# medivhna/TF_Face_Toolbox

Measured on AMD Instinct MI355X. Metric: images/sec (whole node), SphereFaceNet-20 112x112 bs512, higher is better.
Workload: dtype f32; 1 GPU; SphereFaceNet-20 + A-softmax training step, 112x112x3, global batch 512, 10575 classes, Momentum, fp32; global_batch=512, per_gpu_batch=512, parallelism=dp1

## Files before the change

### tf_face_toolbox_amd/csrc/api.hip

```cpp
#include <hip/hip_runtime.h>
#include <stdio.h>
#include <stdlib.h>
#include <string.h>

#include <initializer_list>

#include "../../include/fte.h"
#include "igemm.h"
#include "wgrad16.h"
#include "pw16.h"
#include "kernels.h"
#include "layers.h"
#include "wino.h"
#include "search.h"

namespace {

struct Pads { int out, before; };
inline Pads same_pads(int in, int k, int stride) {
    const int out = (in + stride - 1) / stride;
    int total = (out - 1) * stride + k - in;
    if (total < 0) total = 0;
    return {out, total / 2};
}
// ... 254 lines not shown
inline bool wino_wanted(int n, int h, int wd, int cin, int cout, int ksize, int stride, int op) {
    return !plan_bf16() && !g_plan_bn && wino_sized(n, h, wd, cin, cout, ksize, stride, op);
}
inline bool aligned16(std::initializer_list<const void*> ptrs) {
    uintptr_t v = 0;
    for (const void* q : ptrs) v |= (uintptr_t)q;
    return (v & 15) == 0;
}
struct WinoWs { size_t v_off, u_off, slab_off, total; };
inline WinoWs wino_ws(int n, int h, int wd, int cin, int cout, int op, size_t head) {
    const WinoGeom g = wino_geom(n, h, wd);
    WinoWs w;
    w.v_off = align_up(head);
    if (op == 0) {
        w.u_off = w.v_off + align_up(wino_pack_floats(g.M, cin) * 4);
        w.slab_off = w.total = w.u_off + align_up((size_t)16 * cin * cout * 4);
    } else if (op == 1) {
        w.u_off = w.v_off + align_up(wino_pack_floats(g.M, cout) * 4);
        w.slab_off = w.total = w.u_off + align_up((size_t)16 * cin * cout * 4);
    } else {
        w.u_off = w.v_off + align_up(wino_pack_floats(g.M, cin) * 4);
        w.slab_off = w.u_off;
        w.total = w.slab_off + align_up((size_t)wino_wgrad_splits(cin, cout) * 16 * cin * cout * 4);
    }
    return w;
}
}

extern "C" {

#ifndef FTE_SRC_SHA
#define FTE_SRC_SHA "unstamped"
#endif
const char* fte_version(void) { return "fte 0.2 gfx950 fp32-mfma src:" FTE_SRC_SHA; }
// ... 69 lines not shown
    p.A = (const float*)x;
    p.B = (const float*)w;
    p.c_ld = cout;
    p.Y = y; p.Z = z; p.R = res; p.bias = bias; p.alpha = alpha; p.Y16 = y16;
    p.R16 = res16; p.Z16 = z16;
    int bl = BL_KN;
    if (src16) {
        p.src16 = 1; p.b_ld = cin; bl = BL_NK;
        for (int t = 0; t < ksize * ksize; ++t) p.b_tapoff[t] = t * cout * cin;
    } else {
        p.b_ld = cout;
    }
    if (!set_bytes(&p, (size_t)n * h * wd * cin, (size_t)ksize * ksize * cin * cout, src16 ? 2 : 4)) return FTE_EINVAL;
    if (!src16 && !stat_part && y && wino_wanted(n, h, wd, cin, cout, ksize, stride, 0)) {
        WinoWs wl = wino_ws(n, h, wd, cin, cout, 0, 0);
        if (vpack) { wl.u_off = 0; wl.total = align_up((size_t)16 * cin * cout * 4); }
        if (ws && ws_bytes >= wl.total) {
            if (!aligned16({x, w, bias, alpha, res, z, y, ws, vpack})) return FTE_EINVAL;
            float* V = vpack ? vpack : (float*)((char*)ws + wl.v_off);
            float* U = (float*)((char*)ws + wl.u_off);
            hipError_t e = wino_transform_filter((const float*)w, U, cin, cout, 0, (hipStream_t)stream);
            if (e != hipSuccess) return (int)e;
            e = wino_transform_tiles((const float*)x, V, n, h, wd, cin, 0, (hipStream_t)stream, wino_fwd_small_tiles());
            if (e != hipSuccess) return (int)e;
            WinoMMParams q;
            memset(&q, 0, sizeof(q));
            q.V = V; q.U = U; q.K = cin; q.N = cout; q.g = wino_geom(n, h, wd);
            q.Y = y; q.Z = z; q.R = res; q.bias = bias; q.alpha = alpha;
            return rc(wino_mm(q, EPI_FWD, (hipStream_t)stream));
        }
    }
    if (vpack) return FTE_EWORKSPACE;
    RowPlan rp = plan_rows(p.M, p.N, p.K, ws != nullptr, false, EPI_FWD);
    if (rp.tail_mode >= 2 && ws_bytes < rp.pw_bytes) rp = plan_rows(p.M, p.N, p.K, false);
    if (stat_part) {
        if (rp.tail_mode == 2) return FTE_EINVAL;
        p.SP = stat_part;
        *stat_rows = (int)(rp.main_mtiles + rp.tail_mtiles);
    }
    return rc(launch_rows(p, rp, AL_MK, bl, EPI_FWD, 0, (float*)ws, (hipStream_t)stream));
}
int fte_conv2d_fwd(const float* x, const float* w, const float* bias, const float* alpha, const float* res,
                   float* z, float* y, int n, int h, int wd, int cin, int cout, int ksize, int stride,
// ... 155 lines not shown
        const WinoWs wl = wino_ws(n, h, wd, cin, cout, 1, 2 * half_w + SCRATCH_BYTES);
        if (ws && ws_bytes >= wl.total) {
            if (!aligned16({dz, w, addin, zprev, alpha_prev, raw, dzprev, ws})) return FTE_EINVAL;
            const bool part = zprev && (dalpha_prev || dbias_prev);
            float* V = (float*)((char*)ws + wl.v_off);
            float* U = (float*)((char*)ws + wl.u_off);
            hipError_t e = wino_transform_filter((const float*)w, U, cin, cout, 1, (hipStream_t)stream);
            if (e != hipSuccess) return (int)e;
            e = wino_transform_tiles((const float*)dz, V, n, h, wd, cout, 0, (hipStream_t)stream);
            if (e != hipSuccess) return (int)e;
            WinoMMParams q;
            memset(&q, 0, sizeof(q));
            q.V = V; q.U = U; q.K = cout; q.N = cin; q.g = g;
            q.ADD = addin; q.RAW = raw; q.Zin = zprev; q.alpha = alpha_prev; q.amod = cin; q.DZ = dzprev;
            q.PA = part ? (float*)ws : nullptr; q.PB = part ? (float*)((char*)ws + half_w) : nullptr;
            e = wino_mm(q, EPI_DGRAD, (hipStream_t)stream);
            if (e != hipSuccess) return (int)e;
            if (part) {
                float* scratch = (float*)((char*)ws + 2 * half_w);
                if (dalpha_prev && dbias_prev) return rc(k_reduce_rows2(q.PA, dalpha_prev, q.PB, dbias_prev, nullptr, 1, g.MB, cin, 1, 1.f, scratch, (hipStream_t)stream));
                if (dalpha_prev) return rc(k_reduce_rows(q.PA, dalpha_prev, nullptr, 1, g.MB, cin, 1, 1.f, scratch, (hipStream_t)stream));
                return rc(k_reduce_rows(q.PB, dbias_prev, nullptr, 1, g.MB, cin, 1, 1.f, scratch, (hipStream_t)stream));
            }
            return FTE_OK;
        }
    }
    DgradClass cls[4];
    const int nc = dgrad_classes(n, h, wd, cin, cout, ksize, stride, cls);
    const bool merged = dgrad_mergeable(cls, nc, n, cin);
    long rows = 0;
// ... 1144 lines not shown
```

### tf_face_toolbox_amd/csrc/wino.h

```cpp
#pragma once
#include <hip/hip_runtime.h>
#include <stddef.h>

struct WinoGeom {
    int n, h, w, th, tw;
    long M;
    int MB;
};
WinoGeom wino_geom(int n, int h, int w);

inline size_t wino_pack_floats(long rows, int c) { return (size_t)((rows + 63) / 64) * 64 * (size_t)c * 16; }

hipError_t wino_transform_tiles(const float* x, float* pack, int n, int h, int w, int c, int mode, hipStream_t st, bool small = false);
hipError_t wino_transform_filter(const float* w, float* pack, int cin, int cout, int dgrad, hipStream_t st);

struct WinoMMParams {
    const float* V;
    const float* U;
    int K, N;
    WinoGeom g;
    float* Y; float* Z; const float* R; const float* bias; const float* alpha;
    const float* ADD; float* RAW; const float* Zin; float* DZ; float* PA; float* PB;
    int amod;
};
hipError_t wino_mm(const WinoMMParams& p, int epi, hipStream_t st);

int wino_wgrad_splits(int cin, int cout);
hipError_t wino_wgrad(const float* V, const float* dz, float* slabs, float* dw, const WinoGeom& g, int cin, int cout, hipStream_t st);

void wino_set_algo(int a);
int wino_get_algo();
```

### tf_face_toolbox_amd/csrc/wino.hip

```cpp
#include <hip/hip_runtime.h>
#include <stdint.h>
#include <stdio.h>
#include <stdlib.h>
#include <string.h>

#include <atomic>

#include "igemm.h"
#include "igemm_dev.h"
#include "wino.h"

#ifdef FTE_WINO_STAMP
__device__ unsigned long long* g_wino_stamp = nullptr;
extern "C" int fte_debug_set_wino_stamp(void* buf) {
    return (int)hipMemcpyToSymbol(HIP_SYMBOL(g_wino_stamp), &buf, sizeof(buf));
}
#endif

namespace {

using namespace igemm_dev;

typedef __attribute__((address_space(3))) void lds_void;
__device__ __forceinline__ void dma16(const __amdgpu_buffer_rsrc_t& r, char* lds, unsigned voff, unsigned soff) {
// ... 85 lines not shown
        p[1][b] = 0.5f * (g[0][b] + g[1][b] + g[2][b]);
        p[2][b] = 0.5f * (g[0][b] - g[1][b] + g[2][b]);
        p[3][b] = g[2][b];
    }
    const int KS = K >> 3, rb = row >> 6, r = row & 63, c8 = k & 7;
    float* o = pack + ((((size_t)rb * KS + (k >> 3)) * 16) * 64 + r) * 8 + (((c8 >> 2) ^ ((r >> 4) & 1)) << 2) + (c8 & 3);
#pragma unroll
    for (int i = 0; i < 4; ++i) {
        o[(size_t)(4 * i + 0) * 512] = p[i][0];
        o[(size_t)(4 * i + 1) * 512] = 0.5f * (p[i][0] + p[i][1] + p[i][2]);
        o[(size_t)(4 * i + 2) * 512] = 0.5f * (p[i][0] - p[i][1] + p[i][2]);
        o[(size_t)(4 * i + 3) * 512] = p[i][2];
    }
}

template <int EPI, int NWN>
__global__ __launch_bounds__(256 * NWN, 1) void wino_mm_kernel(const WinoMMParams p, int NBX, int GRP, int vid0, int nvirt) {
    constexpr int NW = 4 * NWN;
    constexpr int BSTG = NWN * (SLAB_B / 2);
    constexpr int STG = SLAB_B + BSTG;
    extern __shared__ __attribute__((aligned(16))) char wsm[];
    const int tid = threadIdx.x;
    const int lane = tid & 63;
    const int wid = __builtin_amdgcn_readfirstlane(tid >> 6);
    const int q = wid & 1, mi = (wid >> 1) & 1, ni = NWN == 2 ? wid >> 2 : 0;
    const int hb = NWN == 2 ? 0 : (int)(blockIdx.x & 1);
    const int li = lane & 31, lh = lane >> 5;
    const int KS = p.K >> 3, NB = p.N >> 6;
    auto decode = [&](int vid, int& mb, int& nb) -> bool {
        if (GRP > 0) {
            const int xcd = vid & 7, slot = vid >> 3;
            const int grp = xcd % GRP, cls = xcd / GRP, C = 8 / GRP;
            mb = (slot / NBX) * C + cls;
            nb = grp * NBX + slot % NBX;
        } else {
            mb = vid / NB; nb = vid - mb * NB;
        }
        return mb < p.g.MB;
    };
    auto next_valid = [&](int vid, int& mb, int& nb) -> int {
        if constexpr (NWN == 2) {
            for (; vid < nvirt; vid += (int)gridDim.x)
                if (decode(vid, mb, nb)) return vid;
        } else if (vid == vid0) {
            int c = 0;
            for (int v = vid0; v < nvirt; ++v)
                if (decode(v, mb, nb)) {
                    if (c == (int)(blockIdx.x >> 1)) return v;
                    ++c;
                }
        }
        return nvirt;
    };
    const unsigned voff = (unsigned)lane * 16u;
    auto issue = [&](int mb, int nb, int s, int stage) {
        const __amdgpu_buffer_rsrc_t rsA = __builtin_amdgcn_make_buffer_rsrc(const_cast<float*>(p.V + (size_t)mb * KS * SLAB_F), 0, (unsigned)KS * SLAB_B, 0x00020000);
// ... 7 lines not shown
#pragma unroll
        for (int i = 0; i < 4; ++i) {
            const int piece = wid + NW * i;
            dma16(rsB, base + SLAB_B + piece * 1024, voff, (unsigned)(s * SLAB_B + (NWN == 2 ? piece : 2 * piece + hb) * 1024));
        }
    };
    constexpr int BPL = NWN * 1024;
    const int a_off = ((8 * q) * 64 + 32 * mi + li) * 32 + ((lh ^ ((li >> 4) & 1)) << 4);
    const int b_off = (8 * q) * BPL + (32 * ni + li) * 32 + ((lh ^ ((li >> 4) & 1)) << 4);
    float* xb = reinterpret_cast<float*>(wsm + STG);
    int* rowpix = reinterpret_cast<int*>(wsm + 2 * STG);
    int* rowflag = rowpix + 64;
    float* red = reinterpret_cast<float*>(rowflag + 64);

    int mb = 0, nb = 0;
    int vid = next_valid(NWN == 2 ? vid0 + (int)blockIdx.x : vid0, mb, nb);
    if (vid >= nvirt) return;
    f32x4 xa[4], xb4[4], ya[4], yb[4];
    auto read_frags = [&](int stage, int half, f32x4 (&fa)[4], f32x4 (&fb)[4], int t) {
        const char* As = wsm + stage * STG;
        fa[t] = *reinterpret_cast<const f32x4*>(As + a_off + (4 * half + t) * 2048);
        fb[t] = *reinterpret_cast<const f32x4*>(As + SLAB_B + b_off + (4 * half + t) * BPL);
    };
    auto dma_piece = [&](const __amdgpu_buffer_rsrc_t& rsA, const __amdgpu_buffer_rsrc_t& rsB, int s, int stage, int i) {
        char* base = wsm + stage * STG;
        if constexpr (NWN == 2) {
            const int piece = wid + 8 * (i >> 1);
            if (i & 1) dma16(rsB, base + SLAB_B + piece * 1024, voff, (unsigned)(s * SLAB_B + piece * 1024));
            else dma16(rsA, base + piece * 1024, voff, (unsigned)(s * SLAB_B + piece * 1024));
        } else {
            const int piece = wid + 4 * (i & 7);
            if (i >= 8) dma16(rsB, base + SLAB_B + piece * 1024, voff, (unsigned)(s * SLAB_B + (2 * piece + hb) * 1024));
            else dma16(rsA, base + piece * 1024, voff, (unsigned)(s * SLAB_B + piece * 1024));
        }
    };
    constexpr int NDMA = NWN == 2 ? 8 : 12;
    issue(mb, nb, 0, 0);
    issue(mb, nb, 1, 1);
    asm volatile("s_waitcnt vmcnt(0)\n\ts_barrier" ::: "memory");
#pragma unroll
    for (int t = 0; t < 4; ++t) read_frags(0, 0, xa, xb4, t);
    bool first = true;
    while (vid < nvirt) {
        int mb2 = 0, nb2 = 0;
        const int vid2 = NWN == 2 ? next_valid(vid + (int)gridDim.x, mb2, nb2) : nvirt;
        const bool has_next = vid2 < nvirt;
#ifdef FTE_WINO_STAMP
        unsigned long long st0 = 0, sr0 = 0, st1 = 0;
        if (g_wino_stamp) { st0 = __builtin_amdgcn_s_memtime(); sr0 = __builtin_amdgcn_s_memrealtime(); __builtin_amdgcn_s_waitcnt(0xC07F); }
#endif
        f32x16 acc[8];
#pragma unroll
        for (int t = 0; t < 8; ++t)
#pragma unroll
            for (int r = 0; r < 16; ++r) acc[t][r] = 0.f;
        for (int s = 0; s < KS; ++s) {
            const int st = s & 1;
            __builtin_amdgcn_sched_barrier(0);
            static_for<0, 16>([&](auto ic) {
                constexpr int idx = decltype(ic)::value, j = idx >> 2, t = idx & 3;
                acc[t] = __builtin_amdgcn_mfma_f32_32x32x2f32(xa[t][j], xb4[t][j], acc[t], 0, 0, 0);
                if constexpr (idx < 4 && !(WMM_ABL & 2)) read_frags(st, 1, ya, yb, idx);
                __builtin_amdgcn_sched_barrier(0);
            });
            if constexpr (WMM_ABL & 4) asm volatile("s_waitcnt vmcnt(0) lgkmcnt(0)" ::: "memory");
            else if (s == 0 && !first) asm volatile("s_waitcnt vmcnt(16) lgkmcnt(0)\n\ts_barrier" ::: "memory");
            else asm volatile("s_waitcnt vmcnt(0) lgkmcnt(0)\n\ts_barrier" ::: "memory");
            const bool same = s + 2 < KS;
            const bool dma = same || (has_next && s + 2 == KS);
            const int dmb = same ? mb : mb2, dnb = same ? nb : nb2, ds = same ? s + 2 : 0;
            const __amdgpu_buffer_rsrc_t rsA = __builtin_amdgcn_make_buffer_rsrc(const_cast<float*>(p.V + (size_t)dmb * KS * SLAB_F), 0, dma ? (unsigned)KS * SLAB_B : 0u, 0x00020000);
            const __amdgpu_buffer_rsrc_t rsB = __builtin_amdgcn_make_buffer_rsrc(const_cast<float*>(p.U + (size_t)dnb * KS * SLAB_F), 0, dma ? (unsigned)KS * SLAB_B : 0u, 0x00020000);
            if (s == 0 && tid < 64) {
                const int m = mb * 64 + tid;
                int pix = -1, fl = 0;
                if (m < (int)p.g.M) {
                    const int tpi = p.g.th * p.g.tw;
                    const int n = m / tpi, rem = m - n * tpi;
                    const int ty = rem / p.g.tw, tx = rem - ty * p.g.tw;
                    pix = (n * p.g.h + 2 * ty) * p.g.w + 2 * tx;
                    fl = ((2 * ty + 1 < p.g.h) ? 1 : 0) | ((2 * tx + 1 < p.g.w) ? 2 : 0);
                }
                rowpix[tid] = pix; rowflag[tid] = fl;
            }
            __builtin_amdgcn_sched_barrier(0);
            static_for<0, 16>([&](auto ic) {
                constexpr int idx = decltype(ic)::value, j = idx >> 2, t = idx & 3;
                acc[4 + t] = __builtin_amdgcn_mfma_f32_32x32x2f32(ya[t][j], yb[t][j], acc[4 + t], 0, 0, 0);
                if constexpr (idx < 4 && !(WMM_ABL & 2)) read_frags(st ^ 1, 0, xa, xb4, idx);
                if constexpr (idx >= 4 && idx < 4 + NDMA && !(WMM_ABL & 1)) dma_piece(rsA, rsB, ds, st, idx - 4);
                __builtin_amdgcn_sched_barrier(0);
            });
        }
#ifdef FTE_WINO_STAMP
        if (g_wino_stamp) { st1 = __builtin_amdgcn_s_memtime(); __builtin_amdgcn_s_waitcnt(0xC07F); }
#endif
        asm volatile("s_waitcnt vmcnt(0) lgkmcnt(0)\n\ts_barrier" ::: "memory");
// ... 4 lines not shown
        float keep[16][2];
#pragma unroll
        for (int r = 0; r < 16; ++r) {
            const float p00 = acc[0][r] + acc[1][r] + acc[2][r], p01 = acc[1][r] - acc[2][r] - acc[3][r];
            const float p10 = acc[4][r] + acc[5][r] + acc[6][r], p11 = acc[5][r] - acc[6][r] - acc[7][r];
            float s0, s1;
            if (q == 0) { keep[r][0] = p00 + p10; keep[r][1] = p01 + p11; s0 = p10; s1 = p11; }
            else { keep[r][0] = -p00 - p10; keep[r][1] = -p01 - p11; s0 = p00; s1 = p01; }
            xb[(wid * 32 + 2 * r) * 64 + lane_e] = s0;
            xb[(wid * 32 + 2 * r + 1) * 64 + lane_e] = s1;
        }
        __builtin_amdgcn_sched_barrier(0);
        const int prw = lane_e >> 3, pc4 = lane_e & 7;
        const int ch0 = nb * 64 + 32 * (NWN == 2 ? ni : hb) + 4 * pc4;
        unsigned off[2][2][2];
#pragma unroll
        for (int h2 = 0; h2 < 2; ++h2)
#pragma unroll
            for (int j = 0; j < 2; ++j) {
                const int rr = 32 * mi + 16 * h2 + prw + 8 * j;
                const int pix = rowpix[rr], fl = rowflag[rr];
                const bool rowok = pix >= 0 && (q == 0 || (fl & 1));
                const unsigned o = (unsigned)((pix + q * p.g.w) * p.N + ch0) * 4u;
                off[0][h2][j] = rowok ? o : OOB;
                off[1][h2][j] = (rowok && (fl & 2)) ? o + (unsigned)p.N * 4u : OOB;
            }
        const unsigned tbytes = (unsigned)((size_t)p.g.n * p.g.h * p.g.w * p.N * 4);
        auto rsrc_of = [&](const float* q_) { return __builtin_amdgcn_make_buffer_rsrc(const_cast<float*>(q_), 0, q_ ? tbytes : 0u, 0x00020000); };
        auto ld4 = [&](const __amdgpu_buffer_rsrc_t& r_, unsigned o) { return __builtin_bit_cast(f32x4, __builtin_amdgcn_raw_buffer_load_b128(r_, o, 0, 0)); };
        auto st4 = [&](const __amdgpu_buffer_rsrc_t& r_, unsigned o, const f32x4& v) { __builtin_amdgcn_raw_buffer_store_b128(__builtin_bit_cast(u32x4, v), r_, o, 0, 0); };
        f32x4 in0[2][2][2], in1[2][2][2];
        f32x4 bias4 = {0.f, 0.f, 0.f, 0.f}, al4 = {1.f, 1.f, 1.f, 1.f};
        bool act = false;
        if constexpr (EPI == EPI_FWD) {
            const __amdgpu_buffer_rsrc_t rsR = rsrc_of(p.R);
#pragma unroll
            for (int b = 0; b < 2; ++b)
#pragma unroll
                for (int h2 = 0; h2 < 2; ++h2)
#pragma unroll
                    for (int j = 0; j < 2; ++j) in0[b][h2][j] = ld4(rsR, off[b][h2][j]);
            if (p.bias) bias4 = *reinterpret_cast<const f32x4*>(p.bias + ch0);
            act = p.alpha != nullptr;
            if (act) al4 = *reinterpret_cast<const f32x4*>(p.alpha + ch0);
        } else {
            const __amdgpu_buffer_rsrc_t rsA = rsrc_of(p.ADD), rsZ = rsrc_of(p.Zin);
#pragma unroll
            for (int b = 0; b < 2; ++b)
#pragma unroll
                for (int h2 = 0; h2 < 2; ++h2)
#pragma unroll
                    for (int j = 0; j < 2; ++j) { in0[b][h2][j] = ld4(rsA, off[b][h2][j]); in1[b][h2][j] = ld4(rsZ, off[b][h2][j]); }
            act = p.Zin != nullptr;
            if (act) al4 = *reinterpret_cast<const f32x4*>(p.alpha + ch0 % p.amod);
        }
        asm volatile("s_waitcnt lgkmcnt(0)\n\ts_barrier" ::: "memory");
#pragma unroll
        for (int r = 0; r < 16; ++r)
#pragma unroll
            for (int b = 0; b < 2; ++b) keep[r][b] += xb[((wid ^ 1) * 32 + 2 * r + b) * 64 + lane_e];
        asm volatile("s_waitcnt lgkmcnt(0)\n\ts_barrier" ::: "memory");
        if (has_next) issue(mb2, nb2, 1, 1);
        float* patch = reinterpret_cast<float*>(wsm + 2 * STG + 2560) + wid * (16 * 36);
        f32x4 sa4 = {0.f, 0.f, 0.f, 0.f}, sb4 = {0.f, 0.f, 0.f, 0.f};
        const __amdgpu_buffer_rsrc_t rsO0 = rsrc_of(EPI == EPI_FWD ? p.Z : p.RAW), rsO1 = rsrc_of(EPI == EPI_FWD ? p.Y : p.DZ);
#pragma unroll
        for (int b = 0; b < 2; ++b)
#pragma unroll
            for (int h2 = 0; h2 < 2; ++h2) {
                __builtin_amdgcn_wave_barrier();
#pragma unroll
                for (int r8 = 0; r8 < 8; ++r8) patch[((r8 & 3) + 8 * (r8 >> 2) + 4 * lh_e) * 36 + li_e] = keep[8 * h2 + r8][b];
                __builtin_amdgcn_fence(__ATOMIC_RELEASE, "wavefront");
                __builtin_amdgcn_wave_barrier();
#pragma unroll
                for (int j = 0; j < 2; ++j) {
                    f32x4 v = *reinterpret_cast<const f32x4*>(patch + (prw + 8 * j) * 36 + 4 * pc4);
                    const unsigned o = off[b][h2][j];
                    if constexpr (EPI == EPI_FWD) {
                        v += bias4;
                        st4(rsO0, o, v);
#pragma unroll
                        for (int e = 0; e < 4; ++e) v[e] = v[e] > 0.f ? v[e] : al4[e] * v[e];
                        v += in0[b][h2][j];
                        st4(rsO1, o, v);
                    } else {
                        v += in0[b][h2][j];
                        st4(rsO0, o, v);
                        const bool in = o != OOB;
#pragma unroll
                        for (int e = 0; e < 4; ++e) {
                            const float z = act ? in1[b][h2][j][e] : 1.f;
                            sa4[e] += in ? v[e] * fminf(z, 0.f) : 0.f;
                            v[e] *= prelu_slope(z, al4[e]);
                            sb4[e] += in ? v[e] : 0.f;
                        }
                        st4(rsO1, o, v);
                    }
                }
            }
        if constexpr (EPI == EPI_DGRAD) {
            if (p.PA) {
#pragma unroll
                for (int e = 0; e < 4; ++e) {
                    float a_ = sa4[e], b_ = sb4[e];
                    a_ += __shfl_xor(a_, 8); b_ += __shfl_xor(b_, 8);
                    a_ += __shfl_xor(a_, 16); b_ += __shfl_xor(b_, 16);
                    a_ += __shfl_xor(a_, 32); b_ += __shfl_xor(b_, 32);
                    if (prw == 0) { red[wid * 32 + 4 * pc4 + e] = a_; red[(NW + wid) * 32 + 4 * pc4 + e] = b_; }
                }
                asm volatile("s_waitcnt lgkmcnt(0)\n\ts_barrier" ::: "memory");
                if (tid < 32 * NWN) {
                    const int n2 = tid >> 5, l2 = tid & 31;
                    float a = 0.f, b = 0.f;
#pragma unroll
                    for (int k = 0; k < 4; ++k) { a += red[(4 * n2 + k) * 32 + l2]; b += red[(NW + 4 * n2 + k) * 32 + l2]; }
                    const size_t o = (size_t)mb * p.N + nb * 64 + (NWN == 2 ? tid : 32 * hb + tid);
                    p.PA[o] = a;
                    if (p.PB) p.PB[o] = b;
                }
            }
        }
#ifdef FTE_WINO_STAMP
        if (g_wino_stamp && tid == 0) {
            const unsigned long long t2 = __builtin_amdgcn_s_memtime(), r2 = __builtin_amdgcn_s_memrealtime();
            unsigned long long* o = g_wino_stamp + 8 * (size_t)vid;
            o[0] = st1 - st0; o[1] = t2 - st1; o[2] = t2 - st0; o[3] = r2 - sr0; o[4] = sr0; o[5] = (unsigned long long)KS; o[6] = blockIdx.x; o[7] = r2;
        }
#endif
        if (has_next) {
#pragma unroll
            for (int t = 0; t < 4; ++t) read_frags(0, 0, xa, xb4, t);
        }
        vid = vid2; mb = mb2; nb = nb2;
        first = false;
    }
}

#ifndef WG_ABL
#define WG_ABL 0
#endif
constexpr int WG_KSTRIDE = 4096 + 32;
constexpr int WG_OP = 8 * WG_KSTRIDE;
__global__ __launch_bounds__(512, 1) void wino_wgrad_kernel(const float* __restrict__ V, const float* __restrict__ dz, float* __restrict__ slabs,
                                                            int cin, int cout, WinoGeom g, int S, unsigned dz_bytes) {
    extern __shared__ __attribute__((aligned(16))) char wsm[];
    const int tid = threadIdx.x;
    const int lane = tid & 63;
    const int wid = __builtin_amdgcn_readfirstlane(tid >> 6);
    const int li = lane & 31, lh = lane >> 5;
// ... 171 lines not shown
    const dim3 grid(8 * ((g.MB + 7) / 8) * (small ? 2 : 1), c / 32);
    if (mode == 0 && small) hipLaunchKernelGGL((wino_tiles_kernel<0, 256>), grid, dim3(256), 0, st, x, pack, h, w, c, g.th, g.tw, g.M, g.MB, (unsigned)xb);
    else if (mode == 0) hipLaunchKernelGGL((wino_tiles_kernel<0, 512>), grid, dim3(512), 0, st, x, pack, h, w, c, g.th, g.tw, g.M, g.MB, (unsigned)xb);
    else hipLaunchKernelGGL((wino_tiles_kernel<1, 512>), grid, dim3(512), 0, st, x, pack, h, w, c, g.th, g.tw, g.M, g.MB, (unsigned)xb);
    return hipGetLastError();
}

hipError_t wino_transform_filter(const float* w, float* pack, int cin, int cout, int dgrad, hipStream_t st) {
    if (cin % 64 || cout % 64) return hipErrorInvalidValue;
    const int total = cin * cout;
    hipLaunchKernelGGL(wino_filter_kernel, dim3((total + 255) / 256), dim3(256), 0, st, w, pack, cin, cout, dgrad);
    return hipGetLastError();
}

namespace {
template <int EPI, int NWN>
hipError_t wino_mm_launch(const WinoMMParams& p, int NBX, int GRP, int vid0, int vid1, int grid, int tiles, hipStream_t st) {
    constexpr int NW = 4 * NWN;
    const size_t lds = 2 * ((size_t)SLAB_B + NWN * (SLAB_B / 2)) + 2560 + (size_t)NW * 16 * 36 * 4;
    static std::atomic<unsigned> attr{0u};
    int dev = 0;
    (void)hipGetDevice(&dev);
    const unsigned bit = 1u << (dev & 31);
    if (!(attr.load(std::memory_order_acquire) & bit)) {
        hipError_t e = hipFuncSetAttribute(reinterpret_cast<const void*>(wino_mm_kernel<EPI, NWN>), hipFuncAttributeMaxDynamicSharedMemorySize, (int)lds);
        if (e != hipSuccess) return e;
        attr.fetch_or(bit, std::memory_order_release);
    }
    const int sig[5] = {AL_MK, BL_NK, EPI, 8, 1};
    const double frac = (double)tiles / ((double)p.g.MB * (p.N / 64));
    const double flops = 2.0 * 16.0 * (double)tiles * 64.0 * 64.0 * p.K;
    const double bytes = frac * ((double)wino_pack_floats(p.g.M, p.K) * 4.0 + 16.0 * p.N * p.K * 4.0 + (double)p.g.n * p.g.h * p.g.w * p.N * 4.0 *
                                 (EPI == EPI_FWD ? (1 + (p.Z ? 1 : 0) + (p.R ? 1 : 0)) : (1 + (p.ADD ? 1 : 0) + (p.RAW ? 1 : 0) + (p.Zin ? 1 : 0))));
    const int h = igemm_prof_begin(sig, (int)((long)tiles * 64 / (p.N / 64)), p.N, 16 * p.K, flops, bytes, st);
    hipLaunchKernelGGL((wino_mm_kernel<EPI, NWN>), dim3(grid), dim3(256 * NWN), lds, st, p, NBX, GRP, vid0, vid1);
    igemm_prof_end(h, EPI == EPI_FWD ? (NWN == 2 ? "wino_mm_kernel<0,2>" : "wino_mm_kernel<0,1>") : (NWN == 2 ? "wino_mm_kernel<1,2>" : "wino_mm_kernel<1,1>"), st);
    return hipGetLastError();
}
}

hipError_t wino_mm(const WinoMMParams& p, int epi, hipStream_t st) {
    if (p.K % 64 || p.N % 64 || p.g.MB <= 0) return hipErrorInvalidValue;
    if ((size_t)p.g.n * p.g.h * p.g.w * p.N >= ((size_t)1 << 31)) return hipErrorInvalidValue;
    const int NB = p.N / 64;
    int NBX = NB < 2 ? NB : 2, GRP = NB / NBX;
    static const int plain = getenv("FTE_WINO_PLAIN_ORDER") ? atoi(getenv("FTE_WINO_PLAIN_ORDER")) : 0;
    int nvirt;
    if (plain || NB % NBX || 8 % GRP) { GRP = 0; nvirt = p.g.MB * NB; }
    else { const int C = 8 / GRP; nvirt = 8 * ((p.g.MB + C - 1) / C) * NBX; }
    static int cus = 0;
    if (!cus) {
        int dev = 0;
// ... 1 lines not shown
        if (hipGetDevice(&dev) != hipSuccess || hipGetDeviceProperties(&prop, dev) != hipSuccess) return hipErrorInvalidDevice;
        cus = prop.multiProcessorCount > 8 ? prop.multiProcessorCount / 8 * 8 : 8;
    }
    const int grid = nvirt < cus ? (nvirt + 7) / 8 * 8 : cus;
    static const int halves = getenv("FTE_WINO_HALF_TILES") ? atoi(getenv("FTE_WINO_HALF_TILES")) : 1;
    auto valid = [&](int vid) {
        if (GRP > 0) { const int xcd = vid & 7, slot = vid >> 3, cls = xcd / GRP, C = 8 / GRP; return (slot / NBX) * C + cls < p.g.MB; }
        return vid / NB < p.g.MB;
    };
    const int rounds = (nvirt + grid - 1) / grid, last = grid * (rounds - 1);
    int L = 0;
    for (int v = last; v < nvirt; ++v) L += valid(v) ? 1 : 0;
    const int total = p.g.MB * NB;
    int tail_base = nvirt;
    if (halves && L > 0 && 2 * L <= cus && (rounds == 1 || halves == 2)) tail_base = last;
    hipError_t e = hipSuccess;
    if (tail_base > 0) {
        e = epi == EPI_FWD ? wino_mm_launch<EPI_FWD, 2>(p, NBX, GRP, 0, tail_base, grid, total - (tail_base < nvirt ? L : 0), st)
                           : wino_mm_launch<EPI_DGRAD, 2>(p, NBX, GRP, 0, tail_base, grid, total - (tail_base < nvirt ? L : 0), st);
        if (e != hipSuccess) return e;
    }
    if (tail_base < nvirt)
        e = epi == EPI_FWD ? wino_mm_launch<EPI_FWD, 1>(p, NBX, GRP, tail_base, nvirt, 2 * L, L, st)
                           : wino_mm_launch<EPI_DGRAD, 1>(p, NBX, GRP, tail_base, nvirt, 2 * L, L, st);
    return e;
}

int wino_wgrad_splits(int cin, int cout) {
    if (cin % 64 || cout % 64) return 0;
    const int P = (cin / 64) * (cout / 64);
    if (P > 256 || 256 % P) return 0;
    return 256 / P;
}

hipError_t wino_wgrad(const float* V, const float* dz, float* slabs, float* dw, const WinoGeom& g, int cin, int cout, hipStream_t st) {
    const int S = wino_wgrad_splits(cin, cout);
    if (!S) return hipErrorInvalidValue;
// ... 39 lines not shown
```

Before: 15220 images/sec.

## Split K across blocks for the Winograd GEMM tail wave with a fixup kernel

Adds a stream-K style path for the last partial wave of the Winograd batched GEMM. Each tail tile's K range is split across several blocks that write partial accumulators to a new workspace region, and a separate fixup kernel sums them and applies the forward or dgrad epilogue. The epilogue code moves into shared device helpers so both kernels can use it. The aim is to fill idle CUs during the tail wave, at the cost of an extra kernel launch, partial-sum traffic through memory, and a larger workspace requirement. That larger requirement could make the Winograd path fall back when the available workspace is small.

```diff
diff --git a/tf_face_toolbox_amd/csrc/api.hip b/tf_face_toolbox_amd/csrc/api.hip
--- a/tf_face_toolbox_amd/csrc/api.hip
+++ b/tf_face_toolbox_amd/csrc/api.hip
@@ -292,10 +292,12 @@
     w.v_off = align_up(head);
     if (op == 0) {
         w.u_off = w.v_off + align_up(wino_pack_floats(g.M, cin) * 4);
-        w.slab_off = w.total = w.u_off + align_up((size_t)16 * cin * cout * 4);
+        w.slab_off = w.u_off + align_up((size_t)16 * cin * cout * 4);
+        w.total = w.slab_off + WINO_KSPLIT_WS_BYTES;
     } else if (op == 1) {
         w.u_off = w.v_off + align_up(wino_pack_floats(g.M, cout) * 4);
-        w.slab_off = w.total = w.u_off + align_up((size_t)16 * cin * cout * 4);
+        w.slab_off = w.u_off + align_up((size_t)16 * cin * cout * 4);
+        w.total = w.slab_off + WINO_KSPLIT_WS_BYTES;
     } else {
         w.u_off = w.v_off + align_up(wino_pack_floats(g.M, cin) * 4);
         w.slab_off = w.u_off;
@@ -395,7 +397,9 @@
     if (!set_bytes(&p, (size_t)n * h * wd * cin, (size_t)ksize * ksize * cin * cout, src16 ? 2 : 4)) return FTE_EINVAL;
     if (!src16 && !stat_part && y && wino_wanted(n, h, wd, cin, cout, ksize, stride, 0)) {
         WinoWs wl = wino_ws(n, h, wd, cin, cout, 0, 0);
-        if (vpack) { wl.u_off = 0; wl.total = align_up((size_t)16 * cin * cout * 4); }
+        if (vpack) {
+            wl.u_off = 0; wl.slab_off = align_up((size_t)16 * cin * cout * 4); wl.total = wl.slab_off + WINO_KSPLIT_WS_BYTES;
+        }
         if (ws && ws_bytes >= wl.total) {
             if (!aligned16({x, w, bias, alpha, res, z, y, ws, vpack})) return FTE_EINVAL;
             float* V = vpack ? vpack : (float*)((char*)ws + wl.v_off);
@@ -408,6 +412,7 @@
             memset(&q, 0, sizeof(q));
             q.V = V; q.U = U; q.K = cin; q.N = cout; q.g = wino_geom(n, h, wd);
             q.Y = y; q.Z = z; q.R = res; q.bias = bias; q.alpha = alpha;
+            q.KW = (float*)((char*)ws + wl.slab_off);
             return rc(wino_mm(q, EPI_FWD, (hipStream_t)stream));
         }
     }
@@ -593,6 +598,7 @@
             q.V = V; q.U = U; q.K = cout; q.N = cin; q.g = g;
             q.ADD = addin; q.RAW = raw; q.Zin = zprev; q.alpha = alpha_prev; q.amod = cin; q.DZ = dzprev;
             q.PA = part ? (float*)ws : nullptr; q.PB = part ? (float*)((char*)ws + half_w) : nullptr;
+            q.KW = (float*)((char*)ws + wl.slab_off);
             e = wino_mm(q, EPI_DGRAD, (hipStream_t)stream);
             if (e != hipSuccess) return (int)e;
             if (part) {
diff --git a/tf_face_toolbox_amd/csrc/wino.h b/tf_face_toolbox_amd/csrc/wino.h
--- a/tf_face_toolbox_amd/csrc/wino.h
+++ b/tf_face_toolbox_amd/csrc/wino.h
@@ -22,7 +22,10 @@
     float* Y; float* Z; const float* R; const float* bias; const float* alpha;
     const float* ADD; float* RAW; const float* Zin; float* DZ; float* PA; float* PB;
     int amod;
+    float* KW;
+    int ksplit;
 };
+constexpr size_t WINO_KSPLIT_WS_BYTES = (size_t)256 * 65536;
 hipError_t wino_mm(const WinoMMParams& p, int epi, hipStream_t st);
 
 int wino_wgrad_splits(int cin, int cout);
diff --git a/tf_face_toolbox_amd/csrc/wino.hip b/tf_face_toolbox_amd/csrc/wino.hip
--- a/tf_face_toolbox_amd/csrc/wino.hip
+++ b/tf_face_toolbox_amd/csrc/wino.hip
@@ -123,8 +123,128 @@
     }
 }
 
-template <int EPI, int NWN>
+
+__device__ __forceinline__ bool wino_decode(const WinoMMParams& p, int NBX, int GRP, int NB, int vid, int& mb, int& nb) {
+    if (GRP > 0) {
+        const int xcd = vid & 7, slot = vid >> 3;
+        const int grp = xcd % GRP, cls = xcd / GRP, C = 8 / GRP;
+        mb = (slot / NBX) * C + cls;
+        nb = grp * NBX + slot % NBX;
+    } else {
+        mb = vid / NB; nb = vid - mb * NB;
+    }
+    return mb < p.g.MB;
+}
+__device__ __forceinline__ void wino_row_entry(const WinoGeom& g, int m, int& pix, int& fl) {
+    pix = -1; fl = 0;
+    if (m < (int)g.M) {
+        const int tpi = g.th * g.tw;
+        const int n = m / tpi, rem = m - n * tpi;
+        const int ty = rem / g.tw, tx = rem - ty * g.tw;
+        pix = (n * g.h + 2 * ty) * g.w + 2 * tx;
+        fl = ((2 * ty + 1 < g.h) ? 1 : 0) | ((2 * tx + 1 < g.w) ? 2 : 0);
+    }
+}
+__device__ __forceinline__ __amdgpu_buffer_rsrc_t wino_rsrc(const float* q, unsigned bytes) {
+    return __builtin_amdgcn_make_buffer_rsrc(const_cast<float*>(q), 0, q ? bytes : 0u, 0x00020000);
+}
+__device__ __forceinline__ f32x4 wino_ld4(const __amdgpu_buffer_rsrc_t& r, unsigned o) {
+    return __builtin_bit_cast(f32x4, __builtin_amdgcn_raw_buffer_load_b128(r, o, 0, 0));
+}
+__device__ __forceinline__ void wino_st4(const __amdgpu_buffer_rsrc_t& r, unsigned o, const f32x4& v) {
+    __builtin_amdgcn_raw_buffer_store_b128(__builtin_bit_cast(u32x4, v), r, o, 0, 0);
+}
+__device__ __forceinline__ void wino_epi_offsets(const WinoMMParams& p, const int* rowpix, const int* rowflag, int q, int mi, int prw, int ch0,
+                                                 unsigned (&off)[2][2][2]) {
+#pragma unroll
+    for (int h2 = 0; h2 < 2; ++h2)
+#pragma unroll
+        for (int j = 0; j < 2; ++j) {
+            const int rr = 32 * mi + 16 * h2 + prw + 8 * j;
+            const int pix = rowpix[rr], fl = rowflag[rr];
+            const bool rowok = pix >= 0 && (q == 0 || (fl & 1));
+            const unsigned o = (unsigned)((pix + q * p.g.w) * p.N + ch0) * 4u;
+            off[0][h2][j] = rowok ? o : OOB;
+            off[1][h2][j] = (rowok && (fl & 2)) ? o + (unsigned)p.N * 4u : OOB;
+        }
+}
+template <int EPI>
+__device__ __forceinline__ void wino_epi_request(const WinoMMParams& p, const unsigned (&off)[2][2][2], int ch0, unsigned tbytes,
+                                                 f32x4 (&in0)[2][2][2], f32x4 (&in1)[2][2][2], f32x4& bias4, f32x4& al4, bool& act) {
+    if constexpr (EPI == EPI_FWD) {
+        const __amdgpu_buffer_rsrc_t rsR = wino_rsrc(p.R, tbytes);
+#pragma unroll
+        for (int b = 0; b < 2; ++b)
+#pragma unroll
+            for (int h2 = 0; h2 < 2; ++h2)
+#pragma unroll
+                for (int j = 0; j < 2; ++j) in0[b][h2][j] = wino_ld4(rsR, off[b][h2][j]);
+        if (p.bias) bias4 = *reinterpret_cast<const f32x4*>(p.bias + ch0);
+        act = p.alpha != nullptr;
+        if (act) al4 = *reinterpret_cast<const f32x4*>(p.alpha + ch0);
+    } else {
+        const __amdgpu_buffer_rsrc_t rsA = wino_rsrc(p.ADD, tbytes), rsZ = wino_rsrc(p.Zin, tbytes);
+#pragma unroll
+        for (int b = 0; b < 2; ++b)
+#pragma unroll
+            for (int h2 = 0; h2 < 2; ++h2)
+#pragma unroll
+                for (int j = 0; j < 2; ++j) { in0[b][h2][j] = wino_ld4(rsA, off[b][h2][j]); in1[b][h2][j] = wino_ld4(rsZ, off[b][h2][j]); }
+        act = p.Zin != nullptr;
+        if (act) al4 = *reinterpret_cast<const f32x4*>(p.alpha + ch0 % p.amod);
+    }
+}
+template <int EPI>
+__device__ __forceinline__ void wino_epi_value(f32x4 v, unsigned o, const f32x4& i0, const f32x4& i1, const f32x4& bias4, const f32x4& al4, bool act,
+                                               const __amdgpu_buffer_rsrc_t& rsO0, const __amdgpu_buffer_rsrc_t& rsO1, f32x4& sa4, f32x4& sb4) {
+    if constexpr (EPI == EPI_FWD) {
+        v += bias4;
+        wino_st4(rsO0, o, v);
+#pragma unroll
+        for (int e = 0; e < 4; ++e) v[e] = v[e] > 0.f ? v[e] : al4[e] * v[e];
+        v += i0;
+        wino_st4(rsO1, o, v);
+    } else {
+        v += i0;
+        wino_st4(rsO0, o, v);
+        const bool in = o != OOB;
+#pragma unroll
+        for (int e = 0; e < 4; ++e) {
+            const float z = act ? i1[e] : 1.f;
+            sa4[e] += in ? v[e] * fminf(z, 0.f) : 0.f;
+            v[e] *= prelu_slope(z, al4[e]);
+            sb4[e] += in ? v[e] : 0.f;
+        }
+        wino_st4(rsO1, o, v);
+    }
+}
+template <int NWN>
+__device__ __forceinline__ void wino_epi_colsums(const WinoMMParams& p, const f32x4& sa4, const f32x4& sb4, float* red, int tid, int wid, int prw,
+                                                 int pc4, int mb, int nb, int hb) {
+    constexpr int NW = 4 * NWN;
+#pragma unroll
+    for (int e = 0; e < 4; ++e) {
+        float a_ = sa4[e], b_ = sb4[e];
+        a_ += __shfl_xor(a_, 8); b_ += __shfl_xor(b_, 8);
+        a_ += __shfl_xor(a_, 16); b_ += __shfl_xor(b_, 16);
+        a_ += __shfl_xor(a_, 32); b_ += __shfl_xor(b_, 32);
+        if (prw == 0) { red[wid * 32 + 4 * pc4 + e] = a_; red[(NW + wid) * 32 + 4 * pc4 + e] = b_; }
+    }
+    asm volatile("s_waitcnt lgkmcnt(0)\n\ts_barrier" ::: "memory");
+    if (tid < 32 * NWN) {
+        const int n2 = tid >> 5, l2 = tid & 31;
+        float a = 0.f, b = 0.f;
+#pragma unroll
+        for (int k = 0; k < 4; ++k) { a += red[(4 * n2 + k) * 32 + l2]; b += red[(NW + 4 * n2 + k) * 32 + l2]; }
+        const size_t o = (size_t)mb * p.N + nb * 64 + (NWN == 2 ? tid : 32 * hb + tid);
+        p.PA[o] = a;
+        if (p.PB) p.PB[o] = b;
+    }
+}
+
+template <int EPI, int NWN, int KSL>
 __global__ __launch_bounds__(256 * NWN, 1) void wino_mm_kernel(const WinoMMParams p, int NBX, int GRP, int vid0, int nvirt) {
+    static_assert(KSL == 0 || NWN == 2, "K slices are slices of whole tiles");
     constexpr int NW = 4 * NWN;
     constexpr int BSTG = NWN * (SLAB_B / 2);
     constexpr int STG = SLAB_B + BSTG;
@@ -136,19 +256,13 @@
     const int hb = NWN == 2 ? 0 : (int)(blockIdx.x & 1);
     const int li = lane & 31, lh = lane >> 5;
     const int KS = p.K >> 3, NB = p.N >> 6;
-    auto decode = [&](int vid, int& mb, int& nb) -> bool {
-        if (GRP > 0) {
-            const int xcd = vid & 7, slot = vid >> 3;
-            const int grp = xcd % GRP, cls = xcd / GRP, C = 8 / GRP;
-            mb = (slot / NBX) * C + cls;
-            nb = grp * NBX + slot % NBX;
-        } else {
-            mb = vid / NB; nb = vid - mb * NB;
-        }
-        return mb < p.g.MB;
-    };
+    auto decode = [&](int vid, int& mb, int& nb) -> bool { return wino_decode(p, NBX, GRP, NB, vid, mb, nb); };
+    const int ksl = KSL ? (int)(blockIdx.x >> 3) % p.ksplit : 0;
     auto next_valid = [&](int vid, int& mb, int& nb) -> int {
-        if constexpr (NWN == 2) {
+        if constexpr (KSL) {
+            const int v = vid0 + 8 * ((int)(blockIdx.x >> 3) / p.ksplit) + (int)(blockIdx.x & 7);
+            return (vid == vid0 && v < nvirt && decode(v, mb, nb)) ? v : nvirt;
+        } else if constexpr (NWN == 2) {
             for (; vid < nvirt; vid += (int)gridDim.x)
                 if (decode(vid, mb, nb)) return vid;
         } else if (vid == vid0) {
@@ -186,8 +300,9 @@
     float* red = reinterpret_cast<float*>(rowflag + 64);
 
     int mb = 0, nb = 0;
-    int vid = next_valid(NWN == 2 ? vid0 + (int)blockIdx.x : vid0, mb, nb);
+    int vid = next_valid((NWN == 2 && !KSL) ? vid0 + (int)blockIdx.x : vid0, mb, nb);
     if (vid >= nvirt) return;
+    const int KL = KSL ? KS / p.ksplit : KS, k0 = KSL ? ksl * KL : 0;
     f32x4 xa[4], xb4[4], ya[4], yb[4];
     auto read_frags = [&](int stage, int half, f32x4 (&fa)[4], f32x4 (&fb)[4], int t) {
         const char* As = wsm + stage * STG;
@@ -207,15 +322,15 @@
         }
     };
     constexpr int NDMA = NWN == 2 ? 8 : 12;
-    issue(mb, nb, 0, 0);
-    issue(mb, nb, 1, 1);
+    issue(mb, nb, k0, 0);
+    issue(mb, nb, k0 + 1, 1);
     asm volatile("s_waitcnt vmcnt(0)\n\ts_barrier" ::: "memory");
 #pragma unroll
     for (int t = 0; t < 4; ++t) read_frags(0, 0, xa, xb4, t);
     bool first = true;
     while (vid < nvirt) {
         int mb2 = 0, nb2 = 0;
-        const int vid2 = NWN == 2 ? next_valid(vid + (int)gridDim.x, mb2, nb2) : nvirt;
+        const int vid2 = (NWN == 2 && !KSL) ? next_valid(vid + (int)gridDim.x, mb2, nb2) : nvirt;
         const bool has_next = vid2 < nvirt;
 #ifdef FTE_WINO_STAMP
         unsigned long long st0 = 0, sr0 = 0, st1 = 0;
@@ -226,7 +341,7 @@
         for (int t = 0; t < 8; ++t)
 #pragma unroll
             for (int r = 0; r < 16; ++r) acc[t][r] = 0.f;
-        for (int s = 0; s < KS; ++s) {
+        for (int s = 0; s < KL; ++s) {
             const int st = s & 1;
             __builtin_amdgcn_sched_barrier(0);
             static_for<0, 16>([&](auto ic) {
@@ -238,21 +353,14 @@
             if constexpr (WMM_ABL & 4) asm volatile("s_waitcnt vmcnt(0) lgkmcnt(0)" ::: "memory");
             else if (s == 0 && !first) asm volatile("s_waitcnt vmcnt(16) lgkmcnt(0)\n\ts_barrier" ::: "memory");
             else asm volatile("s_waitcnt vmcnt(0) lgkmcnt(0)\n\ts_barrier" ::: "memory");
-            const bool same = s + 2 < KS;
-            const bool dma = same || (has_next && s + 2 == KS);
-            const int dmb = same ? mb : mb2, dnb = same ? nb : nb2, ds = same ? s + 2 : 0;
+            const bool same = s + 2 < KL;
+            const bool dma = same || (has_next && s + 2 == KL);
+            const int dmb = same ? mb : mb2, dnb = same ? nb : nb2, ds = same ? k0 + s + 2 : 0;
             const __amdgpu_buffer_rsrc_t rsA = __builtin_amdgcn_make_buffer_rsrc(const_cast<float*>(p.V + (size_t)dmb * KS * SLAB_F), 0, dma ? (unsigned)KS * SLAB_B : 0u, 0x00020000);
             const __amdgpu_buffer_rsrc_t rsB = __builtin_amdgcn_make_buffer_rsrc(const_cast<float*>(p.U + (size_t)dnb * KS * SLAB_F), 0, dma ? (unsigned)KS * SLAB_B : 0u, 0x00020000);
-            if (s == 0 && tid < 64) {
-                const int m = mb * 64 + tid;
-                int pix = -1, fl = 0;
-                if (m < (int)p.g.M) {
-                    const int tpi = p.g.th * p.g.tw;
-                    const int n = m / tpi, rem = m - n * tpi;
-                    const int ty = rem / p.g.tw, tx = rem - ty * p.g.tw;
-                    pix = (n * p.g.h + 2 * ty) * p.g.w + 2 * tx;
-                    fl = ((2 * ty + 1 < p.g.h) ? 1 : 0) | ((2 * tx + 1 < p.g.w) ? 2 : 0);
-                }
+            if (!KSL && s == 0 && tid < 64) {
+                int pix, fl;
+                wino_row_entry(p.g, mb * 64 + tid, pix, fl);
                 rowpix[tid] = pix; rowflag[tid] = fl;
             }
             __builtin_amdgcn_sched_barrier(0);
@@ -287,45 +395,13 @@
         const int prw = lane_e >> 3, pc4 = lane_e & 7;
         const int ch0 = nb * 64 + 32 * (NWN == 2 ? ni : hb) + 4 * pc4;
         unsigned off[2][2][2];
-#pragma unroll
-        for (int h2 = 0; h2 < 2; ++h2)
-#pragma unroll
-            for (int j = 0; j < 2; ++j) {
-                const int rr = 32 * mi + 16 * h2 + prw + 8 * j;
-                const int pix = rowpix[rr], fl = rowflag[rr];
-                const bool rowok = pix >= 0 && (q == 0 || (fl & 1));
-                const unsigned o = (unsigned)((pix + q * p.g.w) * p.N + ch0) * 4u;
-                off[0][h2][j] = rowok ? o : OOB;
-                off[1][h2][j] = (rowok && (fl & 2)) ? o + (unsigned)p.N * 4u : OOB;
-            }
         const unsigned tbytes = (unsigned)((size_t)p.g.n * p.g.h * p.g.w * p.N * 4);
-        auto rsrc_of = [&](const float* q_) { return __builtin_amdgcn_make_buffer_rsrc(const_cast<float*>(q_), 0, q_ ? tbytes : 0u, 0x00020000); };
-        auto ld4 = [&](const __amdgpu_buffer_rsrc_t& r_, unsigned o) { return __builtin_bit_cast(f32x4, __builtin_amdgcn_raw_buffer_load_b128(r_, o, 0, 0)); };
-        auto st4 = [&](const __amdgpu_buffer_rsrc_t& r_, unsigned o, const f32x4& v) { __builtin_amdgcn_raw_buffer_store_b128(__builtin_bit_cast(u32x4, v), r_, o, 0, 0); };
         f32x4 in0[2][2][2], in1[2][2][2];
         f32x4 bias4 = {0.f, 0.f, 0.f, 0.f}, al4 = {1.f, 1.f, 1.f, 1.f};
         bool act = false;
-        if constexpr (EPI == EPI_FWD) {
-            const __amdgpu_buffer_rsrc_t rsR = rsrc_of(p.R);
-#pragma unroll
-            for (int b = 0; b < 2; ++b)
-#pragma unroll
-                for (int h2 = 0; h2 < 2; ++h2)
-#pragma unroll
-                    for (int j = 0; j < 2; ++j) in0[b][h2][j] = ld4(rsR, off[b][h2][j]);
-            if (p.bias) bias4 = *reinterpret_cast<const f32x4*>(p.bias + ch0);
-            act = p.alpha != nullptr;
-            if (act) al4 = *reinterpret_cast<const f32x4*>(p.alpha + ch0);
-        } else {
-            const __amdgpu_buffer_rsrc_t rsA = rsrc_of(p.ADD), rsZ = rsrc_of(p.Zin);
-#pragma unroll
-            for (int b = 0; b < 2; ++b)
-#pragma unroll
-                for (int h2 = 0; h2 < 2; ++h2)
-#pragma unroll
-                    for (int j = 0; j < 2; ++j) { in0[b][h2][j] = ld4(rsA, off[b][h2][j]); in1[b][h2][j] = ld4(rsZ, off[b][h2][j]); }
-            act = p.Zin != nullptr;
-            if (act) al4 = *reinterpret_cast<const f32x4*>(p.alpha + ch0 % p.amod);
+        if constexpr (!KSL) {
+            wino_epi_offsets(p, rowpix, rowflag, q, mi, prw, ch0, off);
+            wino_epi_request<EPI>(p, off, ch0, tbytes, in0, in1, bias4, al4, act);
         }
         asm volatile("s_waitcnt lgkmcnt(0)\n\ts_barrier" ::: "memory");
 #pragma unroll
@@ -336,7 +412,8 @@
         if (has_next) issue(mb2, nb2, 1, 1);
         float* patch = reinterpret_cast<float*>(wsm + 2 * STG + 2560) + wid * (16 * 36);
         f32x4 sa4 = {0.f, 0.f, 0.f, 0.f}, sb4 = {0.f, 0.f, 0.f, 0.f};
-        const __amdgpu_buffer_rsrc_t rsO0 = rsrc_of(EPI == EPI_FWD ? p.Z : p.RAW), rsO1 = rsrc_of(EPI == EPI_FWD ? p.Y : p.DZ);
+        const __amdgpu_buffer_rsrc_t rsO0 = wino_rsrc(EPI == EPI_FWD ? p.Z : p.RAW, tbytes), rsO1 = wino_rsrc(EPI == EPI_FWD ? p.Y : p.DZ, tbytes);
+        f32x4* part = KSL ? reinterpret_cast<f32x4*>(p.KW) + ((size_t)(vid - vid0) * p.ksplit + ksl) * 4096 + wid * 64 + lane_e : nullptr;
 #pragma unroll
         for (int b = 0; b < 2; ++b)
 #pragma unroll
@@ -348,51 +425,13 @@
                 __builtin_amdgcn_wave_barrier();
 #pragma unroll
                 for (int j = 0; j < 2; ++j) {
-                    f32x4 v = *reinterpret_cast<const f32x4*>(patch + (prw + 8 * j) * 36 + 4 * pc4);
-                    const unsigned o = off[b][h2][j];
-                    if constexpr (EPI == EPI_FWD) {
-                        v += bias4;
-                        st4(rsO0, o, v);
-#pragma unroll
-                        for (int e = 0; e < 4; ++e) v[e] = v[e] > 0.f ? v[e] : al4[e] * v[e];
-                        v += in0[b][h2][j];
-                        st4(rsO1, o, v);
-                    } else {
-                        v += in0[b][h2][j];
-                        st4(rsO0, o, v);
-                        const bool in = o != OOB;
-#pragma unroll
-                        for (int e = 0; e < 4; ++e) {
-                            const float z = act ? in1[b][h2][j][e] : 1.f;
-                            sa4[e] += in ? v[e] * fminf(z, 0.f) : 0.f;
-                            v[e] *= prelu_slope(z, al4[e]);
-                            sb4[e] += in ? v[e] : 0.f;
-                        }
-                        st4(rsO1, o, v);
-                    }
+                    const f32x4 v = *reinterpret_cast<const f32x4*>(patch + (prw + 8 * j) * 36 + 4 * pc4);
+                    if constexpr (KSL) part[(4 * b + 2 * h2 + j) * 512] = v;
+                    else wino_epi_value<EPI>(v, off[b][h2][j], in0[b][h2][j], in1[b][h2][j], bias4, al4, act, rsO0, rsO1, sa4, sb4);
                 }
             }
-        if constexpr (EPI == EPI_DGRAD) {
-            if (p.PA) {
-#pragma unroll
-                for (int e = 0; e < 4; ++e) {
-                    float a_ = sa4[e], b_ = sb4[e];
-                    a_ += __shfl_xor(a_, 8); b_ += __shfl_xor(b_, 8);
-                    a_ += __shfl_xor(a_, 16); b_ += __shfl_xor(b_, 16);
-                    a_ += __shfl_xor(a_, 32); b_ += __shfl_xor(b_, 32);
-                    if (prw == 0) { red[wid * 32 + 4 * pc4 + e] = a_; red[(NW + wid) * 32 + 4 * pc4 + e] = b_; }
-                }
-                asm volatile("s_waitcnt lgkmcnt(0)\n\ts_barrier" ::: "memory");
-                if (tid < 32 * NWN) {
-                    const int n2 = tid >> 5, l2 = tid & 31;
-                    float a = 0.f, b = 0.f;
-#pragma unroll
-                    for (int k = 0; k < 4; ++k) { a += red[(4 * n2 + k) * 32 + l2]; b += red[(NW + 4 * n2 + k) * 32 + l2]; }
-                    const size_t o = (size_t)mb * p.N + nb * 64 + (NWN == 2 ? tid : 32 * hb + tid);
-                    p.PA[o] = a;
-                    if (p.PB) p.PB[o] = b;
-                }
-            }
+        if constexpr (EPI == EPI_DGRAD && !KSL) {
+            if (p.PA) wino_epi_colsums<NWN>(p, sa4, sb4, red, tid, wid, prw, pc4, mb, nb, hb);
         }
 #ifdef FTE_WINO_STAMP
         if (g_wino_stamp && tid == 0) {
@@ -407,6 +446,51 @@
         }
         vid = vid2; mb = mb2; nb = nb2;
         first = false;
+    }
+}
+
+template <int EPI>
+__global__ __launch_bounds__(512) void wino_mm_fixup_kernel(const WinoMMParams p, int NBX, int GRP, int vid0, int nvirt) {
+    __shared__ int rowpix[64], rowflag[64];
+    __shared__ float red[2 * 8 * 32];
+    const int tid = threadIdx.x, lane = tid & 63;
+    const int wid = __builtin_amdgcn_readfirstlane(tid >> 6);
+    const int q = wid & 1, mi = (wid >> 1) & 1, ni = wid >> 2;
+    const int vid = vid0 + (int)blockIdx.x;
+    int mb = 0, nb = 0;
+    if (vid >= nvirt || !wino_decode(p, NBX, GRP, p.N >> 6, vid, mb, nb)) return;
+    if (tid < 64) {
+        int pix, fl;
+        wino_row_entry(p.g, mb * 64 + tid, pix, fl);
+        rowpix[tid] = pix; rowflag[tid] = fl;
+    }
+    __syncthreads();
+    const int prw = lane >> 3, pc4 = lane & 7;
+    const int ch0 = nb * 64 + 32 * ni + 4 * pc4;
+    const unsigned tbytes = (unsigned)((size_t)p.g.n * p.g.h * p.g.w * p.N * 4);
+    unsigned off[2][2][2];
+    f32x4 in0[2][2][2], in1[2][2][2];
+    f32x4 bias4 = {0.f, 0.f, 0.f, 0.f}, al4 = {1.f, 1.f, 1.f, 1.f};
+    bool act = false;
+    wino_epi_offsets(p, rowpix, rowflag, q, mi, prw, ch0, off);
+    wino_epi_request<EPI>(p, off, ch0, tbytes, in0, in1, bias4, al4, act);
+    const int S = p.ksplit;
+    const f32x4* part = reinterpret_cast<const f32x4*>(p.KW) + (size_t)blockIdx.x * S * 4096 + tid;
+    f32x4 sa4 = {0.f, 0.f, 0.f, 0.f}, sb4 = {0.f, 0.f, 0.f, 0.f};
+    const __amdgpu_buffer_rsrc_t rsO0 = wino_rsrc(EPI == EPI_FWD ? p.Z : p.RAW, tbytes), rsO1 = wino_rsrc(EPI == EPI_FWD ? p.Y : p.DZ, tbytes);
+#pragma unroll
+    for (int b = 0; b < 2; ++b)
+#pragma unroll
+        for (int h2 = 0; h2 < 2; ++h2)
+#pragma unroll
+            for (int j = 0; j < 2; ++j) {
+                const f32x4* src = part + (4 * b + 2 * h2 + j) * 512;
+                f32x4 v = src[0];
+                for (int s = 1; s < S; ++s) v += src[(size_t)s * 4096];
+                wino_epi_value<EPI>(v, off[b][h2][j], in0[b][h2][j], in1[b][h2][j], bias4, al4, act, rsO0, rsO1, sa4, sb4);
+            }
+    if constexpr (EPI == EPI_DGRAD) {
+        if (p.PA) wino_epi_colsums<2>(p, sa4, sb4, red, tid, wid, prw, pc4, mb, nb, 0);
     }
 }
 
@@ -608,7 +692,7 @@
 }
 
 namespace {
-template <int EPI, int NWN>
+template <int EPI, int NWN, int KSL = 0>
 hipError_t wino_mm_launch(const WinoMMParams& p, int NBX, int GRP, int vid0, int vid1, int grid, int tiles, hipStream_t st) {
     constexpr int NW = 4 * NWN;
     const size_t lds = 2 * ((size_t)SLAB_B + NWN * (SLAB_B / 2)) + 2560 + (size_t)NW * 16 * 36 * 4;
@@ -617,19 +701,25 @@
     (void)hipGetDevice(&dev);
     const unsigned bit = 1u << (dev & 31);
     if (!(attr.load(std::memory_order_acquire) & bit)) {
-        hipError_t e = hipFuncSetAttribute(reinterpret_cast<const void*>(wino_mm_kernel<EPI, NWN>), hipFuncAttributeMaxDynamicSharedMemorySize, (int)lds);
+        hipError_t e = hipFuncSetAttribute(reinterpret_cast<const void*>(wino_mm_kernel<EPI, NWN, KSL>), hipFuncAttributeMaxDynamicSharedMemorySize, (int)lds);
         if (e != hipSuccess) return e;
         attr.fetch_or(bit, std::memory_order_release);
     }
-    const int sig[5] = {AL_MK, BL_NK, EPI, 8, 1};
+    const int sig[5] = {AL_MK, BL_NK, EPI, 8, KSL ? p.ksplit : 1};
     const double frac = (double)tiles / ((double)p.g.MB * (p.N / 64));
     const double flops = 2.0 * 16.0 * (double)tiles * 64.0 * 64.0 * p.K;
     const double bytes = frac * ((double)wino_pack_floats(p.g.M, p.K) * 4.0 + 16.0 * p.N * p.K * 4.0 + (double)p.g.n * p.g.h * p.g.w * p.N * 4.0 *
                                  (EPI == EPI_FWD ? (1 + (p.Z ? 1 : 0) + (p.R ? 1 : 0)) : (1 + (p.ADD ? 1 : 0) + (p.RAW ? 1 : 0) + (p.Zin ? 1 : 0))));
     const int h = igemm_prof_begin(sig, (int)((long)tiles * 64 / (p.N / 64)), p.N, 16 * p.K, flops, bytes, st);
-    hipLaunchKernelGGL((wino_mm_kernel<EPI, NWN>), dim3(grid), dim3(256 * NWN), lds, st, p, NBX, GRP, vid0, vid1);
-    igemm_prof_end(h, EPI == EPI_FWD ? (NWN == 2 ? "wino_mm_kernel<0,2>" : "wino_mm_kernel<0,1>") : (NWN == 2 ? "wino_mm_kernel<1,2>" : "wino_mm_kernel<1,1>"), st);
-    return hipGetLastError();
+    hipLaunchKernelGGL((wino_mm_kernel<EPI, NWN, KSL>), dim3(grid), dim3(256 * NWN), lds, st, p, NBX, GRP, vid0, vid1);
+    igemm_prof_end(h, KSL ? (EPI == EPI_FWD ? "wino_mm_kernel<0,2,1>" : "wino_mm_kernel<1,2,1>")
+                          : EPI == EPI_FWD ? (NWN == 2 ? "wino_mm_kernel<0,2>" : "wino_mm_kernel<0,1>") : (NWN == 2 ? "wino_mm_kernel<1,2>" : "wino_mm_kernel<1,1>"), st);
+    hipError_t e = hipGetLastError();
+    if (KSL && e == hipSuccess) {
+        hipLaunchKernelGGL((wino_mm_fixup_kernel<EPI>), dim3(vid1 - vid0), dim3(512), 0, st, p, NBX, GRP, vid0, vid1);
+        e = hipGetLastError();
+    }
+    return e;
 }
 }
 
@@ -661,13 +751,29 @@
     const int total = p.g.MB * NB;
     int tail_base = nvirt;
     if (halves && L > 0 && 2 * L <= cus && (rounds == 1 || halves == 2)) tail_base = last;
+    constexpr int KSPLIT_MIN_ROUNDS = 3;
+    static const int ksplit = getenv("FTE_WINO_KSPLIT") ? atoi(getenv("FTE_WINO_KSPLIT")) : 1;
+    static const int sk = getenv("FTE_SK") ? atoi(getenv("FTE_SK")) : 1;
+    int S = 0;
+    const int slots = (nvirt - last + 7) / 8 * 8;
+    if (ksplit && sk && p.KW && tail_base == nvirt && rounds > 1 && L > 0 && (ksplit == 2 || (rounds >= KSPLIT_MIN_ROUNDS && 2 * L <= cus))) {
+        const int KS = p.K / 8;
+        for (int s = 2; s <= KS / 4 && slots * s <= cus && (size_t)slots * s * 65536 <= WINO_KSPLIT_WS_BYTES; ++s)
+            if (KS % s == 0) S = s;
+    }
+    if (S >= 2) tail_base = last;
     hipError_t e = hipSuccess;
     if (tail_base > 0) {
         e = epi == EPI_FWD ? wino_mm_launch<EPI_FWD, 2>(p, NBX, GRP, 0, tail_base, grid, total - (tail_base < nvirt ? L : 0), st)
                            : wino_mm_launch<EPI_DGRAD, 2>(p, NBX, GRP, 0, tail_base, grid, total - (tail_base < nvirt ? L : 0), st);
         if (e != hipSuccess) return e;
     }
-    if (tail_base < nvirt)
+    if (tail_base < nvirt && S >= 2) {
+        WinoMMParams ps = p;
+        ps.ksplit = S;
+        e = epi == EPI_FWD ? wino_mm_launch<EPI_FWD, 2, 1>(ps, NBX, GRP, tail_base, nvirt, slots * S, L, st)
+                           : wino_mm_launch<EPI_DGRAD, 2, 1>(ps, NBX, GRP, tail_base, nvirt, slots * S, L, st);
+    } else if (tail_base < nvirt)
         e = epi == EPI_FWD ? wino_mm_launch<EPI_FWD, 1>(p, NBX, GRP, tail_base, nvirt, 2 * L, L, st)
                            : wino_mm_launch<EPI_DGRAD, 1>(p, NBX, GRP, tail_base, nvirt, 2 * L, L, st);
     return e;
```

Result: no change. 15110 images/sec (-0.7%).
